# deepreinforce-ai/CUDA-L2

Measured on AMD Instinct MI355X. Metric: HGEMM TFLOP/s, higher is better.
Workload: dtype f16

## Files before the change

cuda-l2_amd/build.py:

```python
from __future__ import annotations

import concurrent.futures as cf
import hashlib
import os
import shutil
import subprocess
import sys
from pathlib import Path

PKG_DIR = Path(__file__).resolve().parent
REPO_DIR = PKG_DIR.parent
CSRC = PKG_DIR / "csrc"
INCLUDE = REPO_DIR / "include"
BUILD = PKG_DIR / "build"
OBJ = BUILD / "obj"
_SUFFIX = os.environ.get("HGEMM_LIB_SUFFIX", "")
LIB_DIR = PKG_DIR / ("lib_" + _SUFFIX if _SUFFIX else "lib")
BIN_DIR = PKG_DIR / "bin"
ROCM = Path(os.environ.get("ROCM_PATH", "/opt/rocm"))
HIPCC = str(ROCM / "bin" / "hipcc")
ARCH = "gfx950"

LIB_SOURCES = [
    "hgemm_inst_g0.hip",
    "hgemm_inst_g1.hip",
    "hgemm_inst_g2.hip",
    "hgemm_inst_g3.hip",
    "hgemm_inst_g4.hip",
    "hgemm_inst_g5.hip",
    "hgemm_inst_g6.hip",
    "hgemm_inst_g7.hip",
    "hgemm_inst_g8.hip",
    "hgemm_inst_g9.hip",
    "hgemm_inst_g10.hip",
    "hgemm_inst_g11.hip",
    "hgemm_inst_g12.hip",
    "hgemm_inst_g13.hip",
    "hgemm_inst_g14.hip",
    "hgemm_inst_g15.hip",
    "hgemm_inst_g16.hip",
    "hgemm_inst_g17.hip",
    "hgemm_inst_g18.hip",
    "hgemm_registry.hip",
    "hgemm_plan.hip",
    "hgemm_api.hip",
    "hgemm_baselines.hip",
]

HIP_FLAGS = os.environ.get("HGEMM_EXTRA_HIPFLAGS", "").split() + [f"--offload-arch={ARCH}", "-O3", "-std=c++17", "-fPIC", "-Wall", "-Wno-unused-function",
             "-Wno-unused-result", "-Wno-unused-value", "-DROCBLAS_NO_DEPRECATED_WARNINGS", "-D__HIP_PLATFORM_AMD__"]


def _headers_digest() -> str:
    h = hashlib.sha256()
    for d in (CSRC, INCLUDE):
        for p in sorted(d.rglob("*")):
            if p.suffix in (".hpp", ".h", ".def", ".inc"):
                h.update(p.name.encode())
                h.update(p.read_bytes())
    return h.hexdigest()


def _run(cmd: list[str], verbose: bool) -> None:
    if verbose:
        print(" ".join(cmd), flush=True)
    res = subprocess.run(cmd, capture_output=True, text=True)
    if res.returncode != 0:
        sys.stderr.write(res.stdout + res.stderr)
        raise RuntimeError(f"build step failed ({res.returncode}): {' '.join(cmd)}")
    if verbose and (res.stdout or res.stderr):
        print(res.stdout + res.stderr, flush=True)


def compile_object(src: Path, extra_flags: list[str], hdr_digest: str, verbose: bool = False) -> Path:
    OBJ.mkdir(parents=True, exist_ok=True)
    cmd_core = [HIPCC, *HIP_FLAGS, *extra_flags, f"-I{CSRC}", f"-I{INCLUDE}", "-c"]
    key = hashlib.sha256()
    key.update(" ".join(cmd_core).encode())
    key.update(hdr_digest.encode())
    key.update(src.read_bytes())
    obj = OBJ / f"{src.stem}-{key.hexdigest()[:20]}.o"
    if not obj.exists():
        tmp = obj.with_suffix(f".tmp{os.getpid()}.o")
        _run([*cmd_core, str(src), "-o", str(tmp)], verbose)
        os.replace(tmp, obj)
    return obj


def build_library(verbose: bool = False, jobs: int | None = None) -> Path:
    hdr = _headers_digest()
    jobs = jobs or min(8, os.cpu_count() or 1)
    srcs = [CSRC / s for s in LIB_SOURCES]
    with cf.ThreadPoolExecutor(max_workers=jobs) as ex:
        objs = list(ex.map(lambda s: compile_object(s, [], hdr, verbose), srcs))
    LIB_DIR.mkdir(exist_ok=True)
    lib = LIB_DIR / "libhgemm_mi355x.so"
    stamp = LIB_DIR / ".libhgemm_mi355x.stamp"
    want = hashlib.sha256(" ".join(o.name for o in objs).encode()).hexdigest()
    if lib.exists() and stamp.exists() and stamp.read_text() == want:
        return lib
    tmp = lib.with_suffix(f".tmp{os.getpid()}.so")
    _run([HIPCC, f"--offload-arch={ARCH}", "-shared", "-fPIC", *map(str, objs), "-o", str(tmp),
          f"-L{ROCM / 'lib'}", "-lrocblas", "-lhipblaslt", "-lamdhip64",
          "-Wl,--no-undefined", "-Wl,-soname,libhgemm_mi355x.so"], verbose)
    os.replace(tmp, lib)
    stamp.write_text(want)
    return lib


def build_tools(verbose: bool = False) -> list[Path]:
    lib = build_library(verbose)
    hdr = _headers_digest()
    BIN_DIR.mkdir(exist_ok=True)
    out = []
    for name in ("hgemm_tune",):
        src = CSRC / "tools" / f"{name}.cpp"
        if not src.exists():
            continue
        obj = compile_object(src, ["-x", "hip"], hdr, verbose)
        exe = BIN_DIR / name
        stamp = BIN_DIR / f".{name}.stamp"
        want = obj.name + lib.name + str(lib.stat().st_mtime_ns)
        if not (exe.exists() and stamp.exists() and stamp.read_text() == want):
            _run([HIPCC, f"--offload-arch={ARCH}", str(obj), "-o", str(exe), f"-L{LIB_DIR}", "-lhgemm_mi355x",
                  f"-L{ROCM / 'lib'}", "-lamdhip64", "-lrocm_smi64", "-Wl,-rpath,$ORIGIN/../lib", f"-Wl,-rpath,{ROCM / 'lib'}"],
# ... 61 lines not shown
```

cuda-l2_amd/csrc/hgemm_api.hip:

```cpp
#include "hgemm_plan.hpp"
#include "hgemm_kernel_nn.hpp"
#include "hgemm_act.hpp"
#include "../../include/hgemm_mi355x.h"

#include <algorithm>
#include <atomic>
#include <cmath>
#include <cstdint>
#include <cstdlib>
#include <cstring>
#include <mutex>
#include <vector>

using namespace hgemm_mi355x;

namespace {

thread_local int g_last_hip_error = 0;
#ifdef HGEMM_ABLATION
int g_debug_flags = 0;
#endif
#ifdef HGEMM_TIMELINE
unsigned long long* g_timeline = nullptr;
int g_timeline_slots = 0;
// ... 746 lines not shown
  g_ws.clear();
  g_ws_retired.clear();
  return rc;
}

int hgemm_mi355x_release_stream_workspace(void* stream) {
  int dev = 0;
  if (hipGetDevice(&dev) != hipSuccess) return HGEMM_ERR_HIP;
  std::lock_guard<std::mutex> lk(g_ws_mutex);
  for (size_t i = 0; i < g_ws.size(); ++i) {
    if (g_ws[i].device != dev || g_ws[i].stream != (hipStream_t)stream) continue;
    int rc = HGEMM_OK;
    if (g_ws[i].ptr) {
      if (g_ws[i].captured) g_ws_retired.push_back(g_ws[i].ptr);
      else if (hipFree(g_ws[i].ptr) != hipSuccess) rc = HGEMM_ERR_HIP;
    }
    g_ws.erase(g_ws.begin() + (long)i);
    return rc;
  }
  return HGEMM_OK;
}

int hgemm_mi355x_reserve_workspace(int M, int N, int K, void* stream) {
  if (M <= 0 || N <= 0 || K <= 0) return HGEMM_ERR_BAD_ARG;
  int cfg = 0, splits = 1, group = 1;
  const int st = hgemm_mi355x_plan(M, N, K, &cfg, &splits, &group);
  if (st != HGEMM_OK) return st;
  const size_t ws = std::max(hgemm_mi355x_plan_workspace_bytes(cfg, splits, M, N, K), kCounterBytes + (size_t)256 * 256 * 256 * sizeof(float));
  float* slabs = nullptr; unsigned* counters = nullptr;
  const int rc = ensure_workspace(ws - kCounterBytes, (hipStream_t)stream, &slabs, &counters);
  return rc == HGEMM_ERR_NO_WORKSPACE_INTERNAL ? HGEMM_ERR_NO_WORKSPACE : rc;
}

int hgemm_mi355x_launch(int config_id, int splits_arg, int group_m, const void* a, const void* b,
                        const void* b_col_major, void* c, int M, int N, int K, int lda, int ldb,
                        int ldc, void* stream) {
  DisarmTiming disarm_timing;
  if (!a || !c || M <= 0 || N <= 0 || K <= 0) return HGEMM_ERR_BAD_ARG;
  if (config_id >= g_num_kernels || config_id < HGEMM_CONFIG_RAGGED) return HGEMM_ERR_BAD_ARG;
#ifdef HGEMM_TIMELINE
  ++g_timeline_count;
#endif
  hipStream_t s = (hipStream_t)stream;
  const bool aligned = mfma_path_ok(a, b_col_major, c, M, N, K, lda, ldb, ldc);
  unsigned ruled_out = 0;
  auto resolve = [&] {
    return resolve_launch(config_id, splits_arg, group_m, b != nullptr, b_col_major != nullptr, aligned, M, N, K, lda, ldb, ldc, ruled_out);
  };
  LaunchPlan p = resolve();
  float* slabs = nullptr; unsigned* counters = nullptr;
  while (p.status == HGEMM_OK && p.slab_bytes) {
    const int st = ensure_workspace(p.slab_bytes, s, &slabs, &counters);
    if (st == HGEMM_OK) break;
    if (st != HGEMM_ERR_NO_WORKSPACE_INTERNAL && p.form != FORM_HYBRID) return st;
    ruled_out |= 1u << p.form;
    p = resolve();
  }
  if (p.status != HGEMM_OK) return p.status;
  for (int i = 0; i < p.n; ++i) {
    GemmArgs& g = p.d[i].g;
    g.A = (const f16*)a; g.Bt = (const f16*)b_col_major; g.C = (f16*)c;
    if (p.d[i].epi != EPI_C16) {
      g.partial = slabs;
      if (p.counters) g.counters = counters;
    }
    const TimingSlot ts = timing_slot(p.d[i].start, p.d[i].stop);
    switch (p.d[i].thunk) {
      case THUNK_ENTRY: g_kernel_table[config_id].launch(g, p.d[i].grid, s, p.d[i].epi, ts); break;
      case THUNK_SPLITK_REDUCE: launch_splitk_reduce(g.partial, g.C, M, N, ldc, g.splits, s, ts); break;
      case THUNK_TAIL_REDUCE: launch_tail_reduce(g, g_kernel_table[config_id].bm, g_kernel_table[config_id].bn, s, ts); break;
      case THUNK_RAGGED: launch_ragged(g, s, ts); break;
      case THUNK_GENERIC: launch_generic((const f16*)a, (const f16*)b, (f16*)c, M, N, K, lda, N, ldc, s, ts); break;
    }
  }
  hipError_t err = hipGetLastError();
  if (err != hipSuccess) { g_last_hip_error = (int)err; return HGEMM_ERR_HIP; }
  return HGEMM_OK;
}

int hgemm_mi355x_set_one_item_kernel(int on) { return sq_one_set_enabled(on); }

unsigned long long hgemm_mi355x_one_item_kernel_launches(void) { return sq_one_launch_count(); }

int hgemm_mi355x_one_item_kernel_takes(int config_id, int splits, int group_m, int M, int N, int K, int lda, int ldb, int ldc) {
  if (M <= 0 || N <= 0 || K <= 0 || config_id >= g_num_kernels || config_id < HGEMM_CONFIG_RAGGED) return HGEMM_ERR_BAD_ARG;
  const LaunchPlan p = resolve_launch(config_id, splits, group_m, false, true, true, M, N, K, lda, ldb, ldc, 0);
  if (p.status != HGEMM_OK) return p.status;
  static const int q256 = hgemm_mi355x_config_by_name("q256x256_w2x2");
  if (config_id != q256) return 0;
  for (int i = 0; i < p.n; ++i)
    if (p.d[i].thunk == THUNK_ENTRY && sq_one_takes(p.d[i].g, p.d[i].grid, p.d[i].epi)) return 1;
  return 0;
}

int hgemm_mi355x_set_insitu(int enable) {
  const int old = insitu_enabled() ? 1 : 0;
  g_insitu_mode.store(enable ? 1 : 0);
  if (!enable) {
    std::lock_guard<std::mutex> lk(g_insitu_mutex);
    g_insitu.clear();
    g_insitu_epoch.fetch_add(1, std::memory_order_release);
  }
  return old;
}

int hgemm_mi355x_insitu_enabled(void) { return insitu_enabled() ? 1 : 0; }

int hgemm_mi355x_insitu_candidates(int M, int N, int K, int config_id[3], int splits[3], int group_m[3]) {
  if (M <= 0 || N <= 0 || K <= 0 || !config_id || !splits || !group_m) return 0;
  PlanTriple c[3];
  const int n = insitu_candidates(M, N, K, c);
  for (int i = 0; i < n; ++i) { config_id[i] = c[i].cfg; splits[i] = c[i].splits; group_m[i] = c[i].group_m; }
  return n;
}

int hgemm_mi355x_insitu_choice(int M, int N, int K, int* config_id, int* splits, int* group_m) {
  PlanTriple p;
  int dev = 0;
  if (hipGetDevice(&dev) != hipSuccess) { (void)hipGetLastError(); dev = 0; }
  if (!config_id || !splits || !group_m || !insitu_lookup(dev, M, N, K, &p)) return 0;
  *config_id = p.cfg; *splits = p.splits; *group_m = p.group_m;
  return 1;
}

int hgemm_mi355x_fp32(const void* a, const void* b, const void* bt, void* c, int M, int N, int K,
                      void* stream) {
  return run(HGEMM_ACC_FP32, a, b, bt, c, M, N, K, stream);
}

int hgemm_mi355x_fp16(const void* a, const void* b, const void* bt, void* c, int M, int N, int K,
                      void* stream) {
  return run(HGEMM_ACC_FP16, a, b, bt, c, M, N, K, stream);
}

int hgemm_mi355x_nn_num_configs(void) { return kLayoutNN.t.count; }
const char* hgemm_mi355x_nn_config_name(int id) { return tr_config_name(kLayoutNN, id); }
int hgemm_mi355x_nn_config_by_name(const char* name) { return tr_config_by_name(kLayoutNN, name); }
int hgemm_mi355x_nn_config_info(int id, int out[8]) { return tr_config_info(kLayoutNN, id, out); }
int hgemm_mi355x_nn_plan(int M, int N, int K, int* nn_config, int* splits) { return tr_plan(kLayoutNN, M, N, K, nn_config, splits); }
int hgemm_mi355x_nn_runs(int nn_config, int M, int N, int K, int lda, int ldb, int ldc) { return tr_runs(kLayoutNN, TR_F16, kOutC16, nn_config, M, N, K, lda, ldb, ldc); }
size_t hgemm_mi355x_nn_plan_workspace_bytes(int nn_config, int splits, int M, int N, int K) {
  return tr_plan_workspace_bytes(kLayoutNN, nn_config, splits, M, N, K);
}
int hgemm_mi355x_nn_reserve_workspace(int M, int N, int K, void* stream) { return tr_reserve_workspace(kLayoutNN, M, N, K, stream); }
int hgemm_mi355x_launch_nn(int nn_config, int splits_arg, const void* a, const void* b, void* c, int M, int N, int K, int lda, int ldb,
                           int ldc, void* stream) {
  return tr_launch(kLayoutNN, TR_F16, kOutC16, nn_config, splits_arg, a, b, nullptr, c, M, N, K, lda, ldb, ldc, stream);
}
int hgemm_mi355x_nn_fp32(const void* a, const void* b, void* c, int M, int N, int K, void* stream) { return tr_run(kLayoutNN, TR_F16, kOutC16, a, b, nullptr, c, M, N, K, stream); }
int hgemm_mi355x_nn_fp16(const void* a, const void* b, void* c, int M, int N, int K, void* stream) { return tr_run(kLayoutNN, TR_F16, kOutC16, a, b, nullptr, c, M, N, K, stream); }
int hgemm_mi355x_selfcheck_launch_nn(int nn_config, int splits, int operands, int M, int N, int K, int lda, int ldb, int ldc, int ruled_out,
                                     long long out[20]) {
  return tr_selfcheck_launch(kLayoutNN, TR_F16, kOutC16, nn_config, splits, operands, M, N, K, lda, ldb, ldc, ruled_out, out);
}

int hgemm_mi355x_ta_num_configs(void) { return kLayoutTA.t.count; }
const char* hgemm_mi355x_ta_config_name(int id) { return tr_config_name(kLayoutTA, id); }
int hgemm_mi355x_ta_config_by_name(const char* name) { return tr_config_by_name(kLayoutTA, name); }
int hgemm_mi355x_ta_config_info(int id, int out[8]) { return tr_config_info(kLayoutTA, id, out); }
int hgemm_mi355x_ta_plan(int M, int N, int K, int* ta_config, int* splits) { return tr_plan(kLayoutTA, M, N, K, ta_config, splits); }
int hgemm_mi355x_ta_runs(int ta_config, int M, int N, int K, int lda, int ldb, int ldc) { return tr_runs(kLayoutTA, TR_F16, kOutC16, ta_config, M, N, K, lda, ldb, ldc); }
size_t hgemm_mi355x_ta_plan_workspace_bytes(int ta_config, int splits, int M, int N, int K) {
  return tr_plan_workspace_bytes(kLayoutTA, ta_config, splits, M, N, K);
}
int hgemm_mi355x_ta_reserve_workspace(int M, int N, int K, void* stream) { return tr_reserve_workspace(kLayoutTA, M, N, K, stream); }
int hgemm_mi355x_launch_ta(int ta_config, int splits_arg, const void* a_col_major, const void* b, void* c, int M, int N, int K, int lda,
                           int ldb, int ldc, void* stream) {
  return tr_launch(kLayoutTA, TR_F16, kOutC16, ta_config, splits_arg, a_col_major, b, nullptr, c, M, N, K, lda, ldb, ldc, stream);
}
int hgemm_mi355x_ta_fp32(const void* a_col_major, const void* b, void* c, int M, int N, int K, void* stream) { return tr_run(kLayoutTA, TR_F16, kOutC16, a_col_major, b, nullptr, c, M, N, K, stream); }
int hgemm_mi355x_ta_fp16(const void* a_col_major, const void* b, void* c, int M, int N, int K, void* stream) { return tr_run(kLayoutTA, TR_F16, kOutC16, a_col_major, b, nullptr, c, M, N, K, stream); }
int hgemm_mi355x_selfcheck_launch_ta(int ta_config, int splits, int operands, int M, int N, int K, int lda, int ldb, int ldc, int ruled_out,
                                     long long out[20]) {
  return tr_selfcheck_launch(kLayoutTA, TR_F16, kOutC16, ta_config, splits, operands, M, N, K, lda, ldb, ldc, ruled_out, out);
}
// ... 336 lines not shown
```

cuda-l2_amd/csrc/hgemm_inst_g13.hip:

```cpp
#include "hgemm_launch.hpp"
#include "hgemm_kernel_sq_one.hpp"

#include <atomic>

namespace hgemm_mi355x {

template __global__ void hgemm_tn_sq_one_kernel<CfgSQOne>(const GemmArgs);

namespace {
#ifdef HGEMM_TIMELINE
std::atomic<int> g_sq_one_on{0};
#else
std::atomic<int> g_sq_one_on{1};
#endif
std::atomic<unsigned long long> g_sq_one_launches{0};
}

int sq_one_set_enabled(int on) { return g_sq_one_on.exchange(on ? 1 : 0); }
unsigned long long sq_one_launch_count() { return g_sq_one_launches.load(); }

bool sq_one_takes(const GemmArgs& g, int grid, int epi) {
  if (!g_sq_one_on.load(std::memory_order_relaxed)) return false;
  if (epi != EPI_C16 || !c_takes_wide_stores(g)) return false;
  if (g.K % (BK * CfgSQOne::KT) != 0 || g.K / BK < SQ_ONE_MIN_STEPS) return false;
  if (g.splits != 1 || g.tail_tiles != 0 || g.items > grid) return false;
  if (g.flags & (ARG_XCD_STAGGER | ARG_PHASE_OFFSET | ARG_PHASE_OFFSET4)) return false;
#ifdef HGEMM_ABLATION
  if (g.debug) return false;
#endif
  return true;
}

bool launch_sq_one(const GemmArgs& g, int grid, hipStream_t stream, int epi, TimingSlot ts) {
  if (!sq_one_takes(g, grid, epi)) return false;
  g_sq_one_launches.fetch_add(1, std::memory_order_relaxed);
  HGEMM_LAUNCH((hgemm_tn_sq_one_kernel<CfgSQOne>), grid, CfgSQOne::THREADS, stream, ts, g);
  return true;
}

}
```

cuda-l2_amd/csrc/hgemm_launch.hpp:

```cpp
#pragma once
#include "hgemm_kernel_rs.hpp"
#include "hgemm_kernel_sq.hpp"
#include "hgemm_kernel_wd.hpp"
#include "hgemm_kernel_lu.hpp"

#include <hip/hip_ext.h>

#include <type_traits>

namespace hgemm_mi355x {

struct LaunchTiming { hipEvent_t start = nullptr, stop = nullptr; };
extern thread_local LaunchTiming t_launch_timing;

struct TimingSlot { hipEvent_t start = nullptr, stop = nullptr; };
inline TimingSlot timing_slot(bool first, bool last) {
  TimingSlot s;
  if (first) { s.start = t_launch_timing.start; t_launch_timing.start = nullptr; }
  if (last) { s.stop = t_launch_timing.stop; t_launch_timing.stop = nullptr; }
  return s;
}

#define HGEMM_LAUNCH(KERNEL, GRID, THREADS, STREAM, SLOT, ...)                                              \
  do {                                                                                                      \
    if ((SLOT).start || (SLOT).stop)                                                                        \
      hipExtLaunchKernelGGL(KERNEL, dim3(GRID), dim3(THREADS), 0, STREAM, (SLOT).start, (SLOT).stop, 0,     \
                            __VA_ARGS__);                                                                   \
    else                                                                                                    \
      hipLaunchKernelGGL(KERNEL, dim3(GRID), dim3(THREADS), 0, STREAM, __VA_ARGS__);                        \
  } while (0)

template <class CFG>
void launch_cfg(const GemmArgs& g, int grid, hipStream_t stream, int epi, TimingSlot ts) {
  if (epi == EPI_STREAMK) {
    if constexpr (CFG::BM * CFG::BN <= 256 * 128) HGEMM_LAUNCH((hgemm_tn_sk_kernel<CFG>), grid, CFG::THREADS, stream, ts, g);
  } else if (epi == EPI_FUSED)
    HGEMM_LAUNCH((hgemm_tn_kernel<CFG, EPI_FUSED>), grid, CFG::THREADS, stream, ts, g);
  else if (epi == EPI_SLAB)
    HGEMM_LAUNCH((hgemm_tn_kernel<CFG, EPI_SLAB>), grid, CFG::THREADS, stream, ts, g);
  else
    HGEMM_LAUNCH((hgemm_tn_kernel<CFG, EPI_C16>), grid, CFG::THREADS, stream, ts, g);
}

inline bool c_takes_wide_stores(const GemmArgs& g) {
  return ((g.N & 7) == 0) && ((g.ldc & 7) == 0) && ((reinterpret_cast<uintptr_t>(g.C) & 15) == 0);
}

template <class CFG>
void launch_sp(const GemmArgs& g, int grid, hipStream_t stream, int epi, TimingSlot ts) {
  const bool wide = c_takes_wide_stores(g);
  if (epi == EPI_FUSED)
    HGEMM_LAUNCH((hgemm_tn_sp_kernel<CFG, SP_EPI_FUSED>), grid, CFG::THREADS, stream, ts, g);
  else if (epi == EPI_SLAB)
    HGEMM_LAUNCH((hgemm_tn_sp_kernel<CFG, SP_EPI_SLAB>), grid, CFG::THREADS, stream, ts, g);
  else if (wide)
    HGEMM_LAUNCH((hgemm_tn_sp_kernel<CFG, SP_EPI_WIDE>), grid, CFG::THREADS, stream, ts, g);
  else
    HGEMM_LAUNCH((hgemm_tn_sp_kernel<CFG, SP_EPI_NARROW>), grid, CFG::THREADS, stream, ts, g);
}

template <class CFG, int FLAG>
void launch_sq_variant(const GemmArgs& g, int grid, hipStream_t stream, int epi, TimingSlot ts) {
  const bool wide = c_takes_wide_stores(g);
  if (epi == EPI_FUSED)
    HGEMM_LAUNCH((hgemm_tn_sq_kernel<CFG, SP_EPI_FUSED | FLAG>), grid, CFG::THREADS, stream, ts, g);
  else if (epi == EPI_SLAB)
    HGEMM_LAUNCH((hgemm_tn_sq_kernel<CFG, SP_EPI_SLAB | FLAG>), grid, CFG::THREADS, stream, ts, g);
  else if (wide)
    HGEMM_LAUNCH((hgemm_tn_sq_kernel<CFG, SP_EPI_WIDE | FLAG>), grid, CFG::THREADS, stream, ts, g);
  else
    HGEMM_LAUNCH((hgemm_tn_sq_kernel<CFG, SP_EPI_NARROW | FLAG>), grid, CFG::THREADS, stream, ts, g);
}

bool launch_sq_one(const GemmArgs& g, int grid, hipStream_t stream, int epi, TimingSlot ts);
bool sq_one_takes(const GemmArgs& g, int grid, int epi);
int sq_one_set_enabled(int on);
unsigned long long sq_one_launch_count();

template <class CFG>
void launch_sq(const GemmArgs& g, int grid, hipStream_t stream, int epi, TimingSlot ts) {
  if constexpr (std::is_same_v<CFG, CfgSQOne>) {
    if (launch_sq_one(g, grid, stream, epi, ts)) return;
  }
  if constexpr (CFG::MI == 16) {
    if (g.K % (BK * CFG::KT) != 0) return launch_sq_variant<CFG, EPI_KTAIL>(g, grid, stream, epi, ts);
    if (g.flags & ARG_XCD_STAGGER) return launch_sq_variant<CFG, EPI_KSTAGGER>(g, grid, stream, epi, ts);
  }
  launch_sq_variant<CFG, 0>(g, grid, stream, epi, ts);
}

template <class CFG, int FLAG>
void launch_rs_variant(const GemmArgs& g, int grid, hipStream_t stream, int epi, TimingSlot ts) {
  if (epi == EPI_FUSED)
    HGEMM_LAUNCH((hgemm_tn_rs_kernel<CFG, EPI_FUSED | FLAG>), grid, CFG::THREADS, stream, ts, g);
  else if (epi == EPI_SLAB)
    HGEMM_LAUNCH((hgemm_tn_rs_kernel<CFG, EPI_SLAB | FLAG>), grid, CFG::THREADS, stream, ts, g);
  else
    HGEMM_LAUNCH((hgemm_tn_rs_kernel<CFG, EPI_C16 | FLAG>), grid, CFG::THREADS, stream, ts, g);
}

template <class CFG>
void launch_rs(const GemmArgs& g, int grid, hipStream_t stream, int epi, TimingSlot ts) {
  if (epi == EPI_STREAMK)
    HGEMM_LAUNCH((hgemm_tn_rs_sk_kernel<CFG>), grid, CFG::THREADS, stream, ts, g);
  else if (g.K % CFG::BKS != 0)
    launch_rs_variant<CFG, EPI_KTAIL>(g, grid, stream, epi, ts);
  else
    launch_rs_variant<CFG, 0>(g, grid, stream, epi, ts);
}

template <class CFG>
void launch_wd(const GemmArgs& g, int grid, hipStream_t stream, int epi, TimingSlot ts) {
  if (epi == EPI_FUSED)
    HGEMM_LAUNCH((hgemm_tn_wd_kernel<CFG, EPI_FUSED>), grid, CFG::THREADS, stream, ts, g);
  else if (epi == EPI_SLAB)
    HGEMM_LAUNCH((hgemm_tn_wd_kernel<CFG, EPI_SLAB>), grid, CFG::THREADS, stream, ts, g);
  else
    HGEMM_LAUNCH((hgemm_tn_wd_kernel<CFG, EPI_C16>), grid, CFG::THREADS, stream, ts, g);
}

template <class CFG>
void launch_lu(const GemmArgs& g, int grid, hipStream_t stream, int epi, TimingSlot ts) {
  if (epi == EPI_SLAB)
    HGEMM_LAUNCH((hgemm_tn_lu_kernel<CFG, EPI_SLAB>), grid, CFG::THREADS, stream, ts, g);
  else
    HGEMM_LAUNCH((hgemm_tn_lu_kernel<CFG, EPI_C16>), grid, CFG::THREADS, stream, ts, g);
}

enum class Family : char { T = 't', S = 's', Q = 'q', R = 'r', W = 'w', U = 'u' };
enum class KTail : char { NONE, PADDED, DIRECT };

struct KernelEntry {
  const char* name;
  Family family;
  int bm, bn, wm, wn, mi, nbuf;
  int threads, lds_bytes;
  void (*launch)(const GemmArgs&, int, hipStream_t, int, TimingSlot);
  int persistent_wgs;
  bool has_fused;
  int kgran;
  KTail ktail;
  int sk_wgs_per_cu;
  bool explicit_only;
};
inline bool w_splits_k(const KernelEntry& e) { return e.family == Family::W && e.wm * e.wn == 1; }

extern const KernelEntry g_kernel_table[];
extern const int g_num_kernels;

void launch_splitk_reduce(const float* partial, f16* C, int M, int N, int ldc, int splits,
                          hipStream_t stream, TimingSlot ts);
void launch_tail_reduce(const GemmArgs& g, int BM, int BN, hipStream_t stream, TimingSlot ts);
void launch_ragged(const GemmArgs& g, hipStream_t stream, TimingSlot ts);
void launch_generic(const f16* A, const f16* B, f16* C, int M, int N, int K, int lda, int ldb,
                    int ldc, hipStream_t stream, TimingSlot ts);

}
```

include/hgemm_mi355x.h:

```cpp
#ifndef HGEMM_MI355X_H_
#define HGEMM_MI355X_H_

#include <stddef.h>

#ifdef __cplusplus
extern "C" {
#endif

typedef enum {
  HGEMM_OK = 0,
  HGEMM_ERR_BAD_ARG = -1,
  HGEMM_ERR_TOO_LARGE = -2,
  HGEMM_ERR_HIP = -3,
  HGEMM_ERR_BACKEND = -4,
  HGEMM_ERR_NOT_READY = -5,
  HGEMM_ERR_NO_ALGO = -6,
  HGEMM_ERR_NO_WORKSPACE = -7
} hgemm_status_t;

typedef enum { HGEMM_ACC_FP32 = 0, HGEMM_ACC_FP16 = 1 } hgemm_acc_t;

#define HGEMM_CONFIG_GENERIC (-1)
#define HGEMM_CONFIG_RAGGED  (-2)

// ... 106 lines not shown
int bgemm_mi355x_launch_tn_bias(int tn_config, int splits, const void* a, const void* b_col_major, const void* bias, void* c,
                                int M, int N, int K, int lda, int ldb, int ldc, void* stream);
int bgemm_mi355x_tn_bias_runs(int tn_config, int M, int N, int K, int lda, int ldb, int ldc);

#define HGEMM_ACT_RELU 1
#define HGEMM_ACT_GELU 2
#define HGEMM_ACT_GELU_TANH 3
int bgemm_mi355x_tn_bias_act(const void* a, const void* b_col_major, const void* bias, void* c, int M, int N, int K, int act, void* stream);
int bgemm_mi355x_launch_tn_bias_act(int tn_config, int splits, const void* a, const void* b_col_major, const void* bias, void* c,
                                    int M, int N, int K, int lda, int ldb, int ldc, int act, void* stream);
int bgemm_mi355x_tn_bias_act_runs(int tn_config, int M, int N, int K, int lda, int ldb, int ldc);

#define HGEMM_ACT_SILU 4
int bgemm_mi355x_tn_gated(const void* a, const void* wg_col_major, const void* wu_col_major, const void* bias_g, const void* bias_u, void* c,
                          int M, int N, int K, int act, void* stream);
int bgemm_mi355x_launch_tn_gated(int tn_config, int splits, const void* a, const void* wg_col_major, const void* wu_col_major,
                                 const void* bias_g, const void* bias_u, void* c, int M, int N, int K, int lda, int ldb, int ldc, int act,
                                 void* stream);
int bgemm_mi355x_tn_gated_runs(int tn_config, int M, int N, int K, int lda, int ldb, int ldc);

int bgemm_mi355x_tn_bias_act_aux(const void* a, const void* b_col_major, const void* bias, void* c, void* z_out, int M, int N, int K, int act,
                                 void* stream);
int bgemm_mi355x_launch_tn_bias_act_aux(int tn_config, int splits, const void* a, const void* b_col_major, const void* bias, void* c,
                                        void* z_out, int M, int N, int K, int lda, int ldb, int ldc, int ldz, int act, void* stream);
int bgemm_mi355x_tn_bias_act_aux_runs(int tn_config, int M, int N, int K, int lda, int ldb, int ldc, int ldz);

int bgemm_mi355x_nn_dact(const void* a, const void* b, const void* z, void* c, int M, int N, int K, int act, void* stream);
int bgemm_mi355x_launch_nn_dact(int nn_config, int splits, const void* a, const void* b, const void* z, void* c, int M, int N, int K,
                                int lda, int ldb, int ldc, int ldz, int act, void* stream);
int bgemm_mi355x_nn_dact_runs(int nn_config, int M, int N, int K, int lda, int ldb, int ldc, int ldz);

int bgemm_mi355x_nn_dact_dbias(const void* a, const void* b, const void* z, void* c, float* db32, int M, int N, int K, int act,
                               int accumulate, void* stream);
int bgemm_mi355x_launch_nn_dact_dbias(int nn_config, int splits, const void* a, const void* b, const void* z, void* c, float* db32, int M,
                                      int N, int K, int lda, int ldb, int ldc, int ldz, int act, int accumulate, void* stream);
int bgemm_mi355x_nn_dact_dbias_runs(int nn_config, int M, int N, int K, int lda, int ldb, int ldc, int ldz);
size_t bgemm_mi355x_nn_dact_dbias_plan_workspace_bytes(int nn_config, int splits, int M, int N, int K);
int bgemm_mi355x_nn_dact_dbias_reserve_workspace(int M, int N, int K, void* stream);

int bgemm_mi355x_colsum_c32(const void* x, float* out32, int M, int N, int ldx, int accumulate, void* stream);

const char* hgemm_mi355x_strerror(int status);
int hgemm_mi355x_last_hip_error(void);
const char* hgemm_mi355x_version(void);

int hgemm_rocblas_init(void);
int hgemm_rocblas_destroy(void);
int hgemm_rocblas_nn(const void* a, const void* b, void* c, int M, int N, int K, int acc, void* stream);
int hgemm_rocblas_tn(const void* a, const void* b_col_major, void* c, int M, int N, int K, int acc, void* stream);
int hgemm_rocblas_ta(const void* a_col_major, const void* b, void* c, int M, int N, int K, int acc, void* stream);
int bgemm_rocblas_nn(const void* a, const void* b, void* c, int M, int N, int K, void* stream);
int bgemm_rocblas_ta(const void* a_col_major, const void* b, void* c, int M, int N, int K, void* stream);
int bgemm_rocblas_tn(const void* a, const void* b_col_major, void* c, int M, int N, int K, void* stream);

int hgemm_hipblaslt_heuristic_init(void);
int hgemm_hipblaslt_heuristic_destroy(void);
int hgemm_hipblaslt_heuristic_nn(const void* a, const void* b, void* c, int M, int N, int K, int acc, void* stream);
int hgemm_hipblaslt_heuristic_tn(const void* a, const void* b_col_major, void* c, int M, int N, int K, int acc, void* stream);

int hgemm_hipblaslt_autotune_init(void);
int hgemm_hipblaslt_autotune_destroy(void);
int hgemm_hipblaslt_autotune_find_best_nn(int M, int N, int K, int acc);
int hgemm_hipblaslt_autotune_find_best_tn(int M, int N, int K, int acc);
int hgemm_hipblaslt_autotune_nn(const void* a, const void* b, void* c, int M, int N, int K, int acc, void* stream);
int hgemm_hipblaslt_autotune_tn(const void* a, const void* b_col_major, void* c, int M, int N, int K, int acc, void* stream);
int hgemm_hipblaslt_autotune_set_cache(const char* path);
int hgemm_hipblaslt_autotune_from_cache(int tn);
int hgemm_hipblaslt_autotune_cache_stats(int* hits, int* misses);
int hgemm_hipblaslt_autotune_candidates(int tn);
double hgemm_hipblaslt_autotune_best_ms(int tn);
int hgemm_hipblaslt_compute16_fallback(int which, int tn);

int hgemm_fill_normal_f16(void* device_ptr, size_t n, unsigned long long seed, void* stream);

void* hgemm_mi355x_event_create(void);
int hgemm_mi355x_event_destroy(void* event);
int hgemm_mi355x_time_next_launch(void* start_event, void* stop_event);
double hgemm_mi355x_event_elapsed_us(void* start_event, void* stop_event);

int hgemm_mi355x_set_one_item_kernel(int on);
unsigned long long hgemm_mi355x_one_item_kernel_launches(void);
int hgemm_mi355x_one_item_kernel_takes(int config_id, int splits, int group_m, int M, int N, int K, int lda, int ldb, int ldc);

#ifdef __cplusplus
}
#endif
#endif
```

Measured before the change: 1458.

## Add strip-mined epilogue variant of one-item square kernel overlapping stores with last MFMAs

```diff
diff --git a/cuda-l2_amd/build.py b/cuda-l2_amd/build.py
--- a/cuda-l2_amd/build.py
+++ b/cuda-l2_amd/build.py
@@ -41,6 +41,7 @@
     "hgemm_inst_g16.hip",
     "hgemm_inst_g17.hip",
     "hgemm_inst_g18.hip",
+    "hgemm_inst_g19.hip",
     "hgemm_registry.hip",
     "hgemm_plan.hip",
     "hgemm_api.hip",
diff --git a/cuda-l2_amd/csrc/hgemm_api.hip b/cuda-l2_amd/csrc/hgemm_api.hip
--- a/cuda-l2_amd/csrc/hgemm_api.hip
+++ b/cuda-l2_amd/csrc/hgemm_api.hip
@@ -852,15 +852,30 @@
 
 unsigned long long hgemm_mi355x_one_item_kernel_launches(void) { return sq_one_launch_count(); }
 
-int hgemm_mi355x_one_item_kernel_takes(int config_id, int splits, int group_m, int M, int N, int K, int lda, int ldb, int ldc) {
+namespace {
+int one_item_query(bool (*takes)(const GemmArgs&, int, int), int config_id, int splits, int group_m, int M, int N, int K, int lda, int ldb,
+                   int ldc) {
   if (M <= 0 || N <= 0 || K <= 0 || config_id >= g_num_kernels || config_id < HGEMM_CONFIG_RAGGED) return HGEMM_ERR_BAD_ARG;
   const LaunchPlan p = resolve_launch(config_id, splits, group_m, false, true, true, M, N, K, lda, ldb, ldc, 0);
   if (p.status != HGEMM_OK) return p.status;
   static const int q256 = hgemm_mi355x_config_by_name("q256x256_w2x2");
   if (config_id != q256) return 0;
   for (int i = 0; i < p.n; ++i)
-    if (p.d[i].thunk == THUNK_ENTRY && sq_one_takes(p.d[i].g, p.d[i].grid, p.d[i].epi)) return 1;
+    if (p.d[i].thunk == THUNK_ENTRY && takes(p.d[i].g, p.d[i].grid, p.d[i].epi)) return 1;
   return 0;
+}
+}
+
+int hgemm_mi355x_one_item_kernel_takes(int config_id, int splits, int group_m, int M, int N, int K, int lda, int ldb, int ldc) {
+  return one_item_query(sq_one_takes, config_id, splits, group_m, M, N, K, lda, ldb, ldc);
+}
+
+int hgemm_mi355x_set_one_item_strip(int on) { return sq_one_strip_set_enabled(on); }
+
+unsigned long long hgemm_mi355x_one_item_strip_launches(void) { return sq_one_strip_launch_count(); }
+
+int hgemm_mi355x_one_item_strip_takes(int config_id, int splits, int group_m, int M, int N, int K, int lda, int ldb, int ldc) {
+  return one_item_query(sq_one_strip_takes, config_id, splits, group_m, M, N, K, lda, ldb, ldc);
 }
 
 int hgemm_mi355x_set_insitu(int enable) {
diff --git a/cuda-l2_amd/csrc/hgemm_inst_g13.hip b/cuda-l2_amd/csrc/hgemm_inst_g13.hip
--- a/cuda-l2_amd/csrc/hgemm_inst_g13.hip
+++ b/cuda-l2_amd/csrc/hgemm_inst_g13.hip
@@ -14,10 +14,21 @@
 std::atomic<int> g_sq_one_on{1};
 #endif
 std::atomic<unsigned long long> g_sq_one_launches{0};
+#ifdef HGEMM_TIMELINE
+std::atomic<int> g_sq_one_strip_on{0};
+#else
+std::atomic<int> g_sq_one_strip_on{1};
+#endif
+std::atomic<unsigned long long> g_sq_one_strip_launches{0};
 }
 
 int sq_one_set_enabled(int on) { return g_sq_one_on.exchange(on ? 1 : 0); }
 unsigned long long sq_one_launch_count() { return g_sq_one_launches.load(); }
+int sq_one_strip_set_enabled(int on) { return g_sq_one_strip_on.exchange(on ? 1 : 0); }
+unsigned long long sq_one_strip_launch_count() { return g_sq_one_strip_launches.load(); }
+bool sq_one_strip_takes(const GemmArgs& g, int grid, int epi) {
+  return g_sq_one_strip_on.load(std::memory_order_relaxed) && sq_one_takes(g, grid, epi);
+}
 
 bool sq_one_takes(const GemmArgs& g, int grid, int epi) {
   if (!g_sq_one_on.load(std::memory_order_relaxed)) return false;
@@ -34,6 +45,11 @@
 bool launch_sq_one(const GemmArgs& g, int grid, hipStream_t stream, int epi, TimingSlot ts) {
   if (!sq_one_takes(g, grid, epi)) return false;
   g_sq_one_launches.fetch_add(1, std::memory_order_relaxed);
+  if (g_sq_one_strip_on.load(std::memory_order_relaxed)) {
+    g_sq_one_strip_launches.fetch_add(1, std::memory_order_relaxed);
+    launch_sq_one_strip(g, grid, stream, ts);
+    return true;
+  }
   HGEMM_LAUNCH((hgemm_tn_sq_one_kernel<CfgSQOne>), grid, CfgSQOne::THREADS, stream, ts, g);
   return true;
 }
diff --git a/cuda-l2_amd/csrc/hgemm_inst_g19.hip b/cuda-l2_amd/csrc/hgemm_inst_g19.hip
--- /dev/null
+++ b/cuda-l2_amd/csrc/hgemm_inst_g19.hip
@@ -0,0 +1,12 @@
+#include "hgemm_launch.hpp"
+#include "hgemm_kernel_sq_one_strip.hpp"
+
+namespace hgemm_mi355x {
+
+template __global__ void hgemm_tn_sq_one_strip_kernel<CfgSQOne>(const GemmArgs);
+
+void launch_sq_one_strip(const GemmArgs& g, int grid, hipStream_t stream, TimingSlot ts) {
+  HGEMM_LAUNCH((hgemm_tn_sq_one_strip_kernel<CfgSQOne>), grid, CfgSQOne::THREADS, stream, ts, g);
+}
+
+}
diff --git a/cuda-l2_amd/csrc/hgemm_kernel_sq_one_strip.hpp b/cuda-l2_amd/csrc/hgemm_kernel_sq_one_strip.hpp
--- /dev/null
+++ b/cuda-l2_amd/csrc/hgemm_kernel_sq_one_strip.hpp
@@ -0,0 +1,268 @@
+#pragma once
+
+#include "hgemm_kernel_sq_one.hpp"
+
+namespace hgemm_mi355x {
+
+#if defined(__HIP_DEVICE_COMPILE__)
+template <class CFG, bool NT>
+__device__ __forceinline__ void sq_one_strip_last_step(const GemmArgs& g, const f16x8 (&fX)[CFG::NFA], const f16x8 (&fY)[CFG::NFA],
+                                                       const f16x8 (&fU)[CFG::NFB], f16x8 (&fV)[CFG::NFB], const char* vsrc, int m_wave,
+                                                       int n_wave, char* stage, char* tl, int tid) {
+  constexpr int FM = CFG::FM, FN = CFG::FN, NG = FN / 4, GROUPS = FM * NG;
+  static_assert(NG == 2 && FN == 8, "two groups of four tiles per row block, one slot plan");
+  using h2 = __attribute__((ext_vector_type(2))) _Float16;
+  using u4 = __attribute__((ext_vector_type(4))) unsigned;
+  int lane = 0;
+  unsigned waddr[4] = {}, raddr = 0, voff[NG] = {}, row8 = 0;
+  __amdgpu_buffer_rsrc_t rsC;
+  auto setup = [&](int part) {
+    if (part == 0) {
+      asm volatile("v_mbcnt_lo_u32_b32 %0, -1, 0\n\tv_mbcnt_hi_u32_b32 %0, -1, %0" : "=v"(lane));
+      const unsigned lds0 = (unsigned)(uintptr_t)(__attribute__((address_space(3))) char*)stage;
+      const int wrow = lane & 15, wq = lane >> 4;
+#pragma unroll
+      for (int jj = 0; jj < 4; ++jj) waddr[jj] = lds0 + wrow * 128 + (((jj * 2 + (wq >> 1)) ^ (wrow & 7)) << 4) + (wq & 1) * 8;
+    } else if (part == 1) {
+      const unsigned lds0 = (unsigned)(uintptr_t)(__attribute__((address_space(3))) char*)stage;
+      const int rrow = lane >> 3, rch = lane & 7;
+      raddr = lds0 + rrow * 128 + ((rch ^ (rrow & 7)) << 4);
+      row8 = (unsigned)g.ldc * 16u;
+    } else if (part == 2) {
+      const uintptr_t caddr = reinterpret_cast<uintptr_t>(g.C + (size_t)m_wave * g.ldc + n_wave);
+      const uintptr_t cuni = ((uintptr_t)(uint32_t)__builtin_amdgcn_readfirstlane((int)(caddr >> 32)) << 32) |
+                             (uint32_t)__builtin_amdgcn_readfirstlane((int)(uint32_t)caddr);
+      const long long rem = ((long long)(g.M - m_wave) * g.ldc - n_wave) * 2;
+      const unsigned range = __builtin_amdgcn_readfirstlane((int)(rem <= 0 ? 0 : rem > 0x7FFFFFFFLL ? 0x7FFFFFFF : rem));
+      rsC = __builtin_amdgcn_make_buffer_rsrc((void*)cuni, 0, (int)range, 0x00020000);
+    } else {
+      const int rrow = lane >> 3, rch = lane & 7;
+#pragma unroll
+      for (int gg = 0; gg < NG; ++gg)
+        voff[gg] = (n_wave + gg * 64 + rch * 8 < g.N) ? (unsigned)(rrow * g.ldc + gg * 64 + rch * 8) * 2u : 0x80000000u;
+    }
+  };
+  u4 rb[2][2];
+  auto write_tile = [&](int k, int jj) {
+    const int x = (k / NG) * FN + (k % NG) * 4 + jj;
+    const f32x4 v = sp_read_acc(x);
+    const h2 lo = {(f16)v[0], (f16)v[1]}, hi = {(f16)v[2], (f16)v[3]};
+    const unsigned long long pk = (unsigned long long)__builtin_bit_cast(unsigned, lo) | ((unsigned long long)__builtin_bit_cast(unsigned, hi) << 32);
+    if (k & 1) asm volatile("ds_write_b64 %0, %1 offset:2048" ::"v"(waddr[jj]), "v"(pk) : "memory");
+    else       asm volatile("ds_write_b64 %0, %1" ::"v"(waddr[jj]), "v"(pk) : "memory");
+  };
+  auto read_group = [&](int k) {
+    if (k & 1) {
+      asm volatile("ds_read_b128 %0, %1 offset:2048" : "=v"(rb[1][0]) : "v"(raddr) : "memory");
+      asm volatile("ds_read_b128 %0, %1 offset:3072" : "=v"(rb[1][1]) : "v"(raddr) : "memory");
+    } else {
+      asm volatile("ds_read_b128 %0, %1" : "=v"(rb[0][0]) : "v"(raddr) : "memory");
+      asm volatile("ds_read_b128 %0, %1 offset:1024" : "=v"(rb[0][1]) : "v"(raddr) : "memory");
+    }
+  };
+  auto store_group = [&](int k) {
+    const int i = k / NG, gg = k % NG, b = k & 1;
+    asm volatile("s_waitcnt lgkmcnt(0)" : "+v"(rb[b][0]), "+v"(rb[b][1])::"memory");
+#pragma unroll
+    for (int h = 0; h < 2; ++h)
+      __builtin_amdgcn_raw_buffer_store_b128(rb[b][h], rsC, voff[gg], (unsigned)(i * 2 + h) * row8, NT ? 2 : 0);
+  };
+
+#pragma unroll
+  for (int i = 0; i < FM; ++i) {
+#pragma unroll
+    for (int n = 0; n < 2 * FN; ++n) {
+      const int h = n / FN, j = n % FN;
+      if (i == 0 && n == FN) {
+        __builtin_amdgcn_sched_barrier(0);
+        __builtin_amdgcn_s_waitcnt(kWaitLgkm0);
+        __builtin_amdgcn_sched_barrier(0);
+      }
+      if (h == 0) sp_mfma_mi<CFG::MI>(i * FN + j, fU[j], fX[i]);
+      else        sp_mfma_mi<CFG::MI>(i * FN + j, fV[j], fY[i]);
+      if (i == 0) {
+        if (n < FN) fV[n] = *(const f16x8*)(vsrc + n * CFG::MI * ROW_BYTES);
+        else if ((n & 1) == 0) setup((n - FN) / 2);
+      } else {
+        const int ka = 2 * (i - 1), kb = ka + 1;
+        if (n >= 3 && n <= 6) write_tile(ka, n - 3);
+        if (n == 6) read_group(ka);
+        if (n >= 7 && n <= 10) write_tile(kb, n - 7);
+        if (n == 10) read_group(kb);
+        if (n == 13) store_group(ka);
+        if (n == 15) store_group(kb);
+      }
+      __builtin_amdgcn_sched_barrier(0);
+    }
+  }
+  HGEMM_TL_STAMP(tl, 4, tid);
+  sp_mfma_drain();
+  __builtin_amdgcn_sched_barrier(0);
+#pragma unroll
+  for (int jj = 0; jj < 4; ++jj) write_tile(GROUPS - 2, jj);
+  read_group(GROUPS - 2);
+#pragma unroll
+  for (int jj = 0; jj < 4; ++jj) write_tile(GROUPS - 1, jj);
+  store_group(GROUPS - 2);
+  read_group(GROUPS - 1);
+  store_group(GROUPS - 1);
+  __builtin_amdgcn_sched_barrier(0);
+}
+#endif
+
+#define SQ1_FRAG(STAGE, OPOFF, H) ((STAGE) + (OPOFF) + foff[H])
+#define SQ1_K_STEP(YS, ZS, LA, EB, LB, EA, VMP, VMQ, NEXT)                                                              \
+  do {                                                                                                                  \
+    char* st  = smem + (step & 1) * CFG::STAGE_BYTES;                                                                   \
+    char* nst = smem + ((step + 1) & 1) * CFG::STAGE_BYTES;                                                             \
+    sq_interval<CFG, 0, LA, EB, VMP, NEXT>(fX, fU, fV, SQ1_FRAG(st, b_base_off, 1), SQ1_FRAG(st, b_base_off, 1),        \
+                                           ZS, SQ1_FRAG(nst, a_base_off, 1), SQ1_FRAG(nst, a_base_off, 1), wave, voffA, voffB, \
+                                           rsA, st, kbA, rsB, st, kbB);                                                 \
+    kbA += ROW_BYTES;                                                                                                   \
+    sq_interval<CFG, 1, LB, EA, VMQ, NEXT>(YS, fV, fX, SQ1_FRAG(nst, a_base_off, 0), SQ1_FRAG(nst, a_base_off, 0),      \
+                                           fU, SQ1_FRAG(nst, b_base_off, 0), SQ1_FRAG(nst, b_base_off, 0), wave, voffA, voffB, \
+                                           rsB, st, kbB, rsA, nst, kbA);                                                \
+    kbB += ROW_BYTES;                                                                                                   \
+    ++step;                                                                                                             \
+  } while (0)
+#define SQ1_FULL_STEP(YS, ZS) SQ1_K_STEP(YS, ZS, true, true, true, true, CFG::NJA + CFG::NJB, CFG::NJA + CFG::NJB, true)
+
+template <class CFG>
+__global__ void __launch_bounds__(CFG::THREADS) hgemm_tn_sq_one_strip_kernel(const GemmArgs g) {
+  prefetch_kernargs<sizeof(GemmArgs)>();
+#if defined(__HIP_DEVICE_COMPILE__)
+  static_assert(CFG::MI == 16 && CFG::KT == 1 && CFG::WGS == 1, "the 16x16x32, K = 64 per stage, one-workgroup-per-CU member");
+  static_assert(sp_staged_ok<CFG>(CFG::LDS_BYTES), "the LDS-staged wide epilogue");
+  constexpr int BM = CFG::BM, BN = CFG::BN, FM = CFG::FM, FN = CFG::FN, MI = CFG::MI;
+  constexpr int NFA = CFG::NFA, NFB = CFG::NFB;
+#ifdef HGEMM_TIMELINE
+  constexpr int TL_EXTRA = 64;
+#else
+  constexpr int TL_EXTRA = 0;
+#endif
+  constexpr int STAGED_BYTES = CFG::NW * SP_STAGED_BYTES_PER_WAVE;
+  __shared__ __attribute__((aligned(1024))) char smem[CFG::LDS_BYTES + 64 + STAGED_BYTES + TL_EXTRA];
+
+  const int tid  = threadIdx.x;
+  HGEMM_TL_STAMP(smem + CFG::LDS_BYTES, 0, tid);
+  HGEMM_TL_REALTIME(smem + CFG::LDS_BYTES, 1, tid);
+  const int lane = tid & 63;
+  const int wave = __builtin_amdgcn_readfirstlane(tid >> 6);
+  const int wave_m = wave / CFG::WN;
+  const int wave_n = wave % CFG::WN;
+
+  const ItemWalk walk = persistent_walk(g.items);
+  if (walk.count == 0) return;
+  const TileCoord tc = map_logical(g, walk.base + walk.first, BM, BN);
+  const int m0 = __builtin_amdgcn_readfirstlane(tc.m0), n0 = __builtin_amdgcn_readfirstlane(tc.n0);
+  const int nk = __builtin_amdgcn_readfirstlane(tc.nk);
+
+  const int lr = lane & (MI - 1), lq = lane / MI, sw = (lr >> 1) & 7;
+  int foff[2];
+#pragma unroll
+  for (int h = 0; h < 2; ++h) foff[h] = lr * ROW_BYTES + (((h * 4 + lq) ^ sw) << 4);
+  const int a_base_off = wave_m * CFG::TM * ROW_BYTES;
+  const int b_base_off = BM * ROW_BYTES + wave_n * CFG::TN * ROW_BYTES;
+
+  sp_reserve_agprs<CFG::AGPRS>();
+
+  static_assert(CFG::NW % 2 == 0, "the swizzle key of a wave's row blocks must not depend on the piece");
+  const uint32_t chunk0 = (uint32_t)((lane & 7) ^ (((wave & 1) << 2) | (lane >> 4)));
+  uint32_t voffA[CFG::PA], voffB[CFG::PB];
+#pragma unroll
+  for (int q = 0; q < CFG::PA; ++q) voffA[q] = ((uint32_t)((wave + q * CFG::NW) * 8 + (lane >> 3)) * (uint32_t)g.lda + chunk0 * 8u) * 2u;
+#pragma unroll
+  for (int q = 0; q < CFG::PB; ++q) voffB[q] = ((uint32_t)((wave + q * CFG::NW) * 8 + (lane >> 3)) * (uint32_t)g.ldb + chunk0 * 8u) * 2u;
+  auto tile_rsrc = [](const f16* base, int row0, int rows, int ld) __attribute__((always_inline)) {
+    const uintptr_t addr = reinterpret_cast<uintptr_t>(base + (size_t)row0 * ld);
+    const uintptr_t uni = ((uintptr_t)(uint32_t)__builtin_amdgcn_readfirstlane((int)(addr >> 32)) << 32) |
+                          (uint32_t)__builtin_amdgcn_readfirstlane((int)(uint32_t)addr);
+    const unsigned long long rem = (unsigned long long)(rows - row0) * (unsigned long long)ld * 2ull;
+    const unsigned range = (unsigned)__builtin_amdgcn_readfirstlane((int)(rem > 0xFFFFFFFFull ? 0xFFFFFFFFu : (unsigned)rem));
+    return __builtin_amdgcn_make_buffer_rsrc((void*)uni, 0, (int)range, 0x00020000);
+  };
+  const __amdgpu_buffer_rsrc_t rsA = tile_rsrc(g.A, m0, g.M, g.lda), rsB = tile_rsrc(g.Bt, n0, g.N, g.ldb);
+  const uint32_t kb0 = (uint32_t)__builtin_amdgcn_readfirstlane(tc.k_begin * 2);
+  HGEMM_TL_STAMP(smem + CFG::LDS_BYTES + 64 + STAGED_BYTES, 0, tid);
+  constexpr int NZ = FM * FN, NPIECE = 2 * (CFG::NJA + CFG::NJB);
+  int zi = 0, pi = 0;
+#pragma unroll
+  for (int s = 0; s < 2; ++s) {
+#pragma unroll
+    for (int p = 0; p < CFG::NJA; ++p) {
+      sq_issue_piece<CFG, 0>(rsA, voffA, smem + s * CFG::STAGE_BYTES, wave, p, kb0 + s * ROW_BYTES);
+      for (++pi; zi < (pi * NZ) / NPIECE; ++zi) sp_zero_acc(zi);
+    }
+#pragma unroll
+    for (int p = 0; p < CFG::NJB; ++p) {
+      sq_issue_piece<CFG, 1>(rsB, voffB, smem + s * CFG::STAGE_BYTES, wave, p, kb0 + s * ROW_BYTES);
+      for (++pi; zi < (pi * NZ) / NPIECE; ++zi) sp_zero_acc(zi);
+    }
+  }
+  __builtin_amdgcn_sched_barrier(0);
+#pragma unroll
+  for (; zi < NZ; ++zi) sp_zero_acc(zi);
+  HGEMM_TL_STAMP(smem + CFG::LDS_BYTES + 64 + STAGED_BYTES, 1, tid);
+  wait_vmcnt<CFG::NJA + CFG::NJB>();
+  __builtin_amdgcn_s_barrier();
+  HGEMM_TL_STAMP(smem + CFG::LDS_BYTES + 64 + STAGED_BYTES, 2, tid);
+
+  f16x8 fX[NFA], fY[NFA], fZ[NFA], fU[NFB], fV[NFB];
+#pragma unroll
+  for (int r = 0; r < NFA; ++r) {
+    fX[r] = *(const f16x8*)(SQ1_FRAG(smem, a_base_off, 0) + r * MI * ROW_BYTES);
+    fY[r] = *(const f16x8*)(SQ1_FRAG(smem, a_base_off, 1) + r * MI * ROW_BYTES);
+  }
+#pragma unroll
+  for (int r = 0; r < NFB; ++r) fU[r] = *(const f16x8*)(SQ1_FRAG(smem, b_base_off, 0) + r * MI * ROW_BYTES);
+  uint32_t kbA = kb0 + 2 * ROW_BYTES, kbB = kb0 + 2 * ROW_BYTES;
+  __builtin_amdgcn_sched_barrier(0);
+  __builtin_amdgcn_s_waitcnt(kWaitLgkm0);
+  sp_sync();
+#pragma unroll
+  for (int p = 0; p < CFG::DA; ++p) sq_issue_piece<CFG, 0>(rsA, voffA, smem, wave, p, kbA);
+
+  int step = 0;
+  HGEMM_TL_STAMP(smem + CFG::LDS_BYTES, 2, tid);
+  HGEMM_TL_STAMP(smem + CFG::LDS_BYTES, 3, tid);
+  if ((nk & 1) == 0) {
+    sq_settle(fX, fY, fU);
+    SQ1_FULL_STEP(fY, fZ);
+#pragma unroll
+    for (int r = 0; r < NFA; ++r) fY[r] = fZ[r];
+  }
+  sq_settle(fX, fY, fU);
+#pragma clang loop unroll(disable)
+  for (int t = step; t + 4 < nk; t += 2) {
+    SQ1_FULL_STEP(fY, fZ);
+    SQ1_FULL_STEP(fZ, fY);
+  }
+  sq_settle(fX, fY, fU);
+  SQ1_K_STEP(fY, fZ, true, true, true, false, CFG::NJA + CFG::NJB, CFG::NJA + CFG::NJB, true);
+  SQ1_K_STEP(fZ, fY, false, false, false, false, CFG::NJB, 0, true);
+
+  const int m_wave = m0 + wave_m * CFG::TM, n_wave = n0 + wave_n * CFG::TN;
+  const char* vsrc = SQ1_FRAG(smem + (step & 1) * CFG::STAGE_BYTES, b_base_off, 1);
+  char* stg = smem + CFG::LDS_BYTES + 64 + wave * SP_STAGED_BYTES_PER_WAVE;
+  ++step;
+  const bool nt = (g.flags & ARG_NT_STORE) != 0;
+  sq_settle(fX, fY, fU);
+  if (nt) sq_one_strip_last_step<CFG, true>(g, fX, fY, fU, fV, vsrc, m_wave, n_wave, stg, smem + CFG::LDS_BYTES, tid);
+  else    sq_one_strip_last_step<CFG, false>(g, fX, fY, fU, fV, vsrc, m_wave, n_wave, stg, smem + CFG::LDS_BYTES, tid);
+#ifdef HGEMM_TIMELINE
+  HGEMM_TL_STAMP(smem + CFG::LDS_BYTES, 5, tid);
+  wait_vmcnt<0>();
+  HGEMM_TL_STAMP(smem + CFG::LDS_BYTES, 6, tid);
+  HGEMM_TL_REALTIME(smem + CFG::LDS_BYTES, 7, tid);
+  sq_timeline_record(g, smem + CFG::LDS_BYTES, smem + CFG::LDS_BYTES + 64 + STAGED_BYTES, step, 1, tid);
+#endif
+#endif
+}
+
+#undef SQ1_FULL_STEP
+#undef SQ1_K_STEP
+#undef SQ1_FRAG
+
+extern template __global__ void hgemm_tn_sq_one_strip_kernel<CfgSQOne>(const GemmArgs);
+
+}
diff --git a/cuda-l2_amd/csrc/hgemm_launch.hpp b/cuda-l2_amd/csrc/hgemm_launch.hpp
--- a/cuda-l2_amd/csrc/hgemm_launch.hpp
+++ b/cuda-l2_amd/csrc/hgemm_launch.hpp
@@ -76,6 +76,10 @@
 bool sq_one_takes(const GemmArgs& g, int grid, int epi);
 int sq_one_set_enabled(int on);
 unsigned long long sq_one_launch_count();
+void launch_sq_one_strip(const GemmArgs& g, int grid, hipStream_t stream, TimingSlot ts);
+bool sq_one_strip_takes(const GemmArgs& g, int grid, int epi);
+int sq_one_strip_set_enabled(int on);
+unsigned long long sq_one_strip_launch_count();
 
 template <class CFG>
 void launch_sq(const GemmArgs& g, int grid, hipStream_t stream, int epi, TimingSlot ts) {
diff --git a/include/hgemm_mi355x.h b/include/hgemm_mi355x.h
--- a/include/hgemm_mi355x.h
+++ b/include/hgemm_mi355x.h
@@ -212,6 +212,10 @@
 unsigned long long hgemm_mi355x_one_item_kernel_launches(void);
 int hgemm_mi355x_one_item_kernel_takes(int config_id, int splits, int group_m, int M, int N, int K, int lda, int ldb, int ldc);
 
+int hgemm_mi355x_set_one_item_strip(int on);
+unsigned long long hgemm_mi355x_one_item_strip_launches(void);
+int hgemm_mi355x_one_item_strip_takes(int config_id, int splits, int group_m, int M, int N, int K, int lda, int ldb, int ldc);
+
 #ifdef __cplusplus
 }
 #endif
```

New measurement: 1471 (median of 6 runs). Within noise of the previous version (+0.9%).
